# ucl-bug/helmnet

Hardware: AMD Instinct MI355X
Metric: solver iterations/sec (whole node), 256^2 domain batch=32 (higher is better)
Workload: dtype f32; 1 GPU; 256x256 ring-phantom SoS maps, batch=32 per GPU, point source [30, 128], shipped jcp checkpoint weights, UNet precision fp32 (BASELINE configs[1]); batch_per_gpu=32, domain=256, lanes=1, unet_precision=fp32, parallelism=dp1 (batch shards, no data-path collective)

## Files before the change

helmnet_amd/_lib.py:

```python
from __future__ import annotations

import ctypes
import os
from ctypes import POINTER, c_char_p, c_double, c_float, c_int, c_int64, c_size_t, c_void_p

import torch

_LIB_PATH = os.environ.get("HELMNET_HIP_LIB") or os.path.join(os.path.dirname(os.path.abspath(__file__)), "libhelmnet_hip.so")
_lib = None

HN_ACT = {"prelu": 0, "relu": 1, "leakyrelu": 2, "celu": 3, "tanh": 4, "gelu": 5, "tanhshrink": 6, "softplus": 7}
HN_PRECISION = {"fp32": 0, "bf16x3": 1, "fp16": 2, "bf16x2": 3, "valu": 4}
HN_OPTION = {"lanes": 0, "side_stream": 1, "deep": 3, "spectral_pfa": 4, "spectral_radix16": 5, "dc_valu": 6, "spectral_cols": 7, "train_fused": 10, "train_overlap": 11, "dc_pair": 12, "side_sync": 13, "state_kernel": 14, "hist_copy": 15, "inc_sigma_map": 16, "spectral_mixed": 17, "f64_fft": 18,
             "graph": 100, "train_lanes": 101, "spectral_plain": 102}
HN_COUNTER = {"graph_replays": 0, "eager_iterations": 1, "graphs_captured": 2, "stream_probes": 3, "side_candidate": 4, "train_fwd_events": 5, "flag_sync_iterations": 6, "spectral_route": 7, "f64_route": 8}
ABI_VERSION = 7
HN_VJP = {"continue": 1, "defer": 2}

SYMBOLS = {
    "hn_abi_version": (c_int, []),
    "hn_create": (c_int, [POINTER(c_void_p), c_int]),
    "hn_destroy": (None, [c_void_p]),
    "hn_last_error": (c_char_p, [c_void_p]),
    "hn_set_unet_precision": (c_int, [c_void_p, c_int]),
    "hn_get_unet_precision": (c_int, [c_void_p]),
    "hn_set_option": (c_int, [c_void_p, c_int, c_int]),
    "hn_get_counter": (c_int64, [c_void_p, c_int]),
    "hn_check_async_errors": (c_int, [c_void_p]),
    "hn_weight_count": (c_size_t, [c_int, c_int, c_int]),
    "hn_load_weights": (c_int, [c_void_p, POINTER(c_float), c_size_t, c_int, c_int, c_int, c_int]),
    "hn_set_domain": (c_int, [c_void_p, c_int, c_int, c_float, c_float]),
    "hn_set_domain_rect": (c_int, [c_void_p, c_int, c_int, c_int, c_float, c_float]),
    "hn_get_sigmas": (c_int, [c_void_p, c_void_p, c_void_p]),
    "hn_state_len": (c_int64, [c_void_p]),
    "hn_reserve": (c_int, [c_void_p, c_int]),
    "hn_laplacian": (c_int, [c_void_p, c_void_p, c_void_p, c_int, c_void_p]),
    "hn_residual": (c_int, [c_void_p, c_void_p, c_void_p, c_void_p, c_int, c_void_p, c_int, c_void_p]),
    "hn_residual_vjp": (c_int, [c_void_p, c_void_p, c_void_p, c_void_p, c_int, c_void_p]),
# ... 90 lines not shown
```

helmnet_amd/csrc/hn_api.hip:

```cpp
#include <cmath>
#include <cstdlib>
#include <cstring>

#include <cstdio>
#include "hn_internal.h"

namespace hn {

static thread_local std::string g_err;

void set_global_error(const char* msg) { g_err = msg; }

int fail(hn_ctx* ctx, int code, const char* fmt, ...) {
    char buf[512];
    va_list ap;
    va_start(ap, fmt);
    vsnprintf(buf, sizeof(buf), fmt, ap);
    va_end(ap);
    if (ctx) ctx->err = buf;
    g_err = buf;
    return code;
}

ProfScope::ProfScope(hn_ctx* ctx, int id, hipStream_t st) : c(ctx), s(st) {
// ... 270 lines not shown
    if (std::strncmp(prop.gcnArchName, "gfx950", 6) != 0)
        return fail(nullptr, HN_ERR_UNSUPPORTED, "device %d is %s; this library is built for gfx950 only", device_id, prop.gcnArchName);
    int prev = -1;
    (void)hipGetDevice(&prev);
    if ((e = hipSetDevice(device_id)) != hipSuccess) return fail(nullptr, HN_ERR_HIP, "hipSetDevice: %s", hipGetErrorString(e));
    if (prev >= 0 && prev != device_id) (void)hipSetDevice(prev);
    hn_ctx* c = new (std::nothrow) hn_ctx();
    if (!c) return fail(nullptr, HN_ERR_NOMEM, "out of host memory");
    c->device = device_id;
    *out = c;
    auto bad_env = [&](const char* name, const char* v) {
        const std::string why = c->err;
        hn_destroy(c);
        *out = nullptr;
        return fail(nullptr, HN_ERR_ARG, "hn_create: environment variable %s=%s rejected (%s)", name, v, why.c_str());
    };
    if (const char* v = getenv("HN_UNET_IMPL")) {
        const int mode = std::strcmp(v, "fp32") == 0 ? HN_PREC_FP32 : std::strcmp(v, "bf16x3") == 0 ? HN_PREC_BF16X3 : std::strcmp(v, "fp16") == 0 ? HN_PREC_FP16
                       : std::strcmp(v, "bf16x2") == 0 ? HN_PREC_BF16X2 : std::strcmp(v, "valu") == 0 ? HN_PREC_FP32_VALU : -1;
        if (hn_set_unet_precision(c, mode) != HN_OK) return bad_env("HN_UNET_IMPL", v);
    }
    const struct { const char* env; int opt; } knobs[] = {{"HN_STREAMS", HN_OPT_LANES}, {"HN_SIDE_STREAM", HN_OPT_SIDE_STREAM},
                                                            {"HN_GRAPH", HN_EXP_GRAPH}, {"HN_DEEP", HN_OPT_DEEP},
                                                            {"HN_TRAIN_LANES", HN_EXP_TRAIN_LANES}, {"HN_TRAIN_FUSED", HN_OPT_TRAIN_FUSED}, {"HN_TRAIN_OVERLAP", HN_OPT_TRAIN_OVERLAP}, {"HN_DC_VALU", HN_OPT_DC_VALU}, {"HN_DC_PAIR", HN_OPT_DC_PAIR}, {"HN_SIDE_SYNC", HN_OPT_SIDE_SYNC}, {"HN_STATE_KERNEL", HN_OPT_STATE_KERNEL}, {"HN_HIST_COPY", HN_OPT_HIST_COPY}, {"HN_INC_SIGMA_MAP", HN_OPT_INC_SIGMA_MAP}, {"HN_SPECTRAL_MIXED", HN_OPT_SPECTRAL_MIXED}, {"HN_F64_FFT", HN_OPT_F64_FFT}, {"HN_SPECTRAL_PLAIN", HN_EXP_SPECTRAL_PLAIN}};
    for (const char* name : {"ROCPROF_COUNTER_COLLECTION", "ROCPROF_COUNTERS", "ROCP_METRICS"})
        if (const char* v = getenv(name))
            if (v[0] != '\0' && std::strcmp(v, "0") != 0 && std::strcmp(v, "False") != 0 && std::strcmp(v, "false") != 0) c->opt_side_sync = 0;
    if (const char* v = getenv("HN_SIDE_PRIORITY")) { const int p = std::atoi(v); c->opt_side_priority = p < 0 || p > 3 ? 0 : p; }
    if (const char* v = getenv("HN_DEFER_JOIN")) c->opt_defer_join = std::atoi(v) != 0;
    for (const auto& k : knobs)
        if (const char* v = getenv(k.env)) {
            char* end = nullptr;
            const long n = std::strtol(v, &end, 10);
            if (end == v || *end != '\0') { c->err = "not an integer"; return bad_env(k.env, v); }
            if (hn_set_option(c, k.opt, (int)n) != HN_OK) return bad_env(k.env, v);
        }
    *out = c;
    return HN_OK;
}

int hn_set_unet_precision(hn_ctx* ctx, int precision) {
    if (!ctx) return HN_ERR_ARG;
    if (precision < HN_PREC_FP32 || precision > HN_PREC_FP32_VALU)
        return fail(ctx, HN_ERR_ARG, "hn_set_unet_precision: unknown mode %d", precision);
    if (precision != ctx->precision) clear_step_graphs(ctx);
    ctx->precision = precision;
    return HN_OK;
// ... 13 lines not shown
            ctx->opt_side_stream = value;
            break;
        case HN_EXP_GRAPH:
            if (value < 0 || value > 64 || (value > 1 && (value & 1)))
                return fail(ctx, HN_ERR_ARG, "HN_EXP_GRAPH must be 0, 1 or an even number of iterations per graph <= 64 (got %d)", value);
            ctx->opt_graph = value;
            break;
        case HN_OPT_DEEP:
            if (value < 0 || value > 2) return fail(ctx, HN_ERR_ARG, "HN_OPT_DEEP must be 0, 1 or 2 (got %d)", value);
            ctx->opt_deep = value;
            break;
        case HN_OPT_SPECTRAL_PFA:
            if (value < 0 || value > 1) return fail(ctx, HN_ERR_ARG, "HN_OPT_SPECTRAL_PFA must be 0 or 1 (got %d)", value);
            ctx->opt_pfa = value;
            break;
        case HN_OPT_SPECTRAL_MIXED:
            if (value < 0 || value > 1) return fail(ctx, HN_ERR_ARG, "HN_OPT_SPECTRAL_MIXED must be 0 or 1 (got %d)", value);
            ctx->opt_mixed = value;
            break;
        case HN_OPT_F64_FFT:
            if (value < 0 || value > 1) return fail(ctx, HN_ERR_ARG, "HN_OPT_F64_FFT must be 0 or 1 (got %d)", value);
            ctx->opt_f64_fft = value;
            break;
        case HN_OPT_DC_VALU:
            if (value < 0 || value > 4) return fail(ctx, HN_ERR_ARG, "HN_OPT_DC_VALU must be 0 .. 4 (got %d)", value);
            ctx->opt_dc_valu = value;
            break;
        case HN_OPT_DC_PAIR:
            if (value < 0 || value > 1) return fail(ctx, HN_ERR_ARG, "HN_OPT_DC_PAIR must be 0 or 1 (got %d)", value);
            ctx->opt_dc_pair = value;
            break;
        case HN_OPT_STATE_KERNEL:
            if (value < 0 || value > 1) return fail(ctx, HN_ERR_ARG, "HN_OPT_STATE_KERNEL must be 0 or 1 (got %d)", value);
            ctx->opt_state_kernel = value;
            break;
        case HN_OPT_INC_SIGMA_MAP:
            if (value < 0 || value > 1) return fail(ctx, HN_ERR_ARG, "HN_OPT_INC_SIGMA_MAP must be 0 or 1 (got %d)", value);
            ctx->opt_inc_sigma_map = value;
            break;
        case HN_OPT_HIST_COPY:
            if (value < 0 || value > 1) return fail(ctx, HN_ERR_ARG, "HN_OPT_HIST_COPY must be 0 or 1 (got %d)", value);
            ctx->opt_hist_copy = value;
            break;
        case HN_OPT_SIDE_SYNC:
            if (value < 0 || value > 1) return fail(ctx, HN_ERR_ARG, "HN_OPT_SIDE_SYNC must be 0 or 1 (got %d)", value);
            ctx->opt_side_sync = value;
// ... 20 lines not shown
            break;
        case HN_OPT_TRAIN_OVERLAP:
            if (value < 0 || value > 2) return fail(ctx, HN_ERR_ARG, "HN_OPT_TRAIN_OVERLAP must be 0, 1 or 2 (got %d)", value);
            ctx->opt_train_overlap = value;
            break;
        default: return fail(ctx, HN_ERR_ARG, "hn_set_option: unknown option %d", option);
    }
    clear_step_graphs(ctx);
    return HN_OK;
}

int64_t hn_get_counter(const hn_ctx* ctx, int counter) {
    if (!ctx) return -1;
    switch (counter) {
        case HN_CNT_GRAPH_REPLAYS: return ctx->graph_replays;
        case HN_CNT_EAGER_ITERATIONS: return ctx->eager_iterations;
        case HN_CNT_GRAPHS_CAPTURED: return ctx->graphs_captured;
        case HN_CNT_STREAM_PROBES: return ctx->probes_run;
        case HN_CNT_TRAIN_FWD_EVENTS: return ctx->train_fwd_events;
        case HN_CNT_FLAG_SYNC_ITERATIONS: return ctx->flag_sync_iterations;
        case HN_CNT_SIDE_CANDIDATE: return ctx->picks[0].known.empty() ? -1 : ctx->picks[0].last_chosen;
        case HN_CNT_SPECTRAL_ROUTE: return ctx->rect != nullptr ? 5 : ctx->tab.n == 0 ? 0 : ctx->tab.pow2 ? 1 : ctx->tab.pfa_p != 0 ? 2 : ctx->tab.mix_p != 0 ? 4 : 3;
        case HN_CNT_F64_ROUTE: return ctx->f64_route;
        default: return -1;
    }
}

void hn_destroy(hn_ctx* ctx) {
    if (!ctx) return;
    DeviceGuard guard(ctx);
    (void)hipDeviceSynchronize();
    clear_step_graphs(ctx);
    if (ctx->cap_stream) (void)hipStreamDestroy(ctx->cap_stream);
    (void)hipFree(ctx->it_counter);
    free_workspace(ctx);
    train_free(ctx);
    unet_f64_free(ctx);
    jvp_free(ctx);
    krylov_free(ctx);
    f64_fft_free(ctx);
    spec_free(ctx->tab);
    spec_rect_free(ctx);
    spec_lossy_free(ctx);
    (void)hipFree(ctx->wdev);
    (void)hipFree(ctx->fragdev);
    for (int j = 0; j < ctx->n_streams; ++j) {
// ... 297 lines not shown

int hn_double_conv(hn_ctx* ctx, const float* x, int cin, int cout, const float* weights_host, int act_kind, float* out,
                   int batch, int h, int w, void* stream) {
    if (!ctx || !x || !weights_host || !out) return fail(ctx, HN_ERR_ARG, "hn_double_conv: NULL argument");
    if (batch < 1 || h < 1 || w < 1) return fail(ctx, HN_ERR_ARG, "hn_double_conv: batch, h, w must be positive");
    if (act_kind < HN_ACT_PRELU || act_kind > HN_ACT_SOFTPLUS) return fail(ctx, HN_ERR_UNSUPPORTED, "activation kind %d is not implemented", act_kind);
    const bool ok = (cout == kFeat && (cin == kInCh || cin == kFeat || cin == kFeat + kState || cin == 2 * kFeat)) || (cout == kState && cin == kFeat + kState);
    if (!ok) return fail(ctx, HN_ERR_UNSUPPORTED, "hn_double_conv: (cin, cout) = (%d, %d) is not one of (6,8) (8,8) (10,8) (16,8) (10,2)", cin, cout);
    DcW dw;
    size_t n_floats = 0;
    const RawDc r = raw_dc(n_floats, cin, cout, cout);
    return with_temp_weights(ctx, n_floats, (hipStream_t)stream,
        [&](std::vector<float>& packed, float* dev) { dw = pack_dc(weights_host, packed.data(), dev, r, act_kind); },
        [&]() { return module_double_conv(ctx, x, cin, cout, dw, out, batch, h, w, (hipStream_t)stream); });
}

int hn_conv8x8(hn_ctx* ctx, const float* x, const float* weights_host, int transposed, float* out, int batch, int h, int w, void* stream) {
    if (!ctx || !x || !weights_host || !out) return fail(ctx, HN_ERR_ARG, "hn_conv8x8: NULL argument");
    if (batch < 1 || h < 1 || w < 1) return fail(ctx, HN_ERR_ARG, "hn_conv8x8: batch, h, w must be positive");
    if (!transposed && ((h | w) & 1)) return fail(ctx, HN_ERR_UNSUPPORTED, "hn_conv8x8: the stride-2 convolution needs even h, w (got %d, %d)", h, w);
    K8W kw;
    size_t n_floats = 0;
    const RawK8 r = raw_k8(n_floats);
    return with_temp_weights(ctx, n_floats, (hipStream_t)stream,
        [&](std::vector<float>& packed, float* dev) { kw = pack_k8(weights_host, packed.data(), dev, r, transposed != 0); },
        [&]() { return module_conv8x8(ctx, x, kw, transposed != 0, out, batch, h, w, (hipStream_t)stream); });
}

int hn_out_conv(hn_ctx* ctx, const float* x, const float* weights_host, float* out, int batch, int h, int w, void* stream) {
    if (!ctx || !x || !weights_host || !out) return fail(ctx, HN_ERR_ARG, "hn_out_conv: NULL argument");
    if (batch < 1 || h < 1 || w < 1) return fail(ctx, HN_ERR_ARG, "hn_out_conv: batch, h, w must be positive");
    const float *dw = nullptr, *db = nullptr;
    return with_temp_weights(ctx, 2 * kFeat + 2, (hipStream_t)stream,
        [&](std::vector<float>& packed, float* dev) {
            repack_oihw(weights_host, packed.data(), 2, kFeat, 1);
            packed[2 * kFeat] = weights_host[2 * kFeat]; packed[2 * kFeat + 1] = weights_host[2 * kFeat + 1];
            dw = dev; db = dev + 2 * kFeat;
        },
        [&]() { return module_out_conv(ctx, x, dw, db, out, batch, h, w, (hipStream_t)stream); });
}

}

namespace hn {
namespace {

struct StepArgs {
    float *wf, *res, *states;
    const float *k_sq, *src;
// ... 397 lines not shown
```

helmnet_amd/csrc/hn_internal.h:

```cpp
#pragma once
#include <hip/hip_runtime.h>

#include <complex>
#include <cstdarg>
#include <cstdint>
#include <cstdio>
#include <string>
#include <vector>

#include "helmnet_hip.h"

namespace hn {

constexpr int kFeat = 8;
constexpr int kCounterStride = 32;
constexpr int kState = 2;
constexpr int kInCh = 6;
constexpr int kMaxDepth = 6;

struct Src {
    const float* p;
    long sb;
    long sc;
    float scale;
// ... 219 lines not shown
    long pair_flags_cap = 0;
    unsigned pair_epoch = 0;
    unsigned* pair_done = nullptr;
    int opt_hist_copy = 0;
    int opt_state_kernel = 1;
    int opt_side_sync = 1;
    unsigned* sync_flags = nullptr;
    unsigned sync_epoch = 0;
    int* sync_err = nullptr;
    int* sync_err_dev = nullptr;
    hn_stream_verdict_rec* stream_tab = nullptr;
    hn_stream_verdict_rec* stream_tab_dev = nullptr;
    int stream_tab_cap = 0;
    float2* inc_sigma_map = nullptr;
    int inc_sigma_band = 0;
    float inc_w_sigma[144]{};
    int opt_inc_sigma_map = 1;
    const float* zero_page = nullptr;
    const float* outc_w = nullptr;
    const float* outc_b = nullptr;
    hn::SpecTables tab;
    hn::F64Fft* f64fft = nullptr;
    int opt_f64_fft = 0;
    int f64_route = 0;
    hn::RectDomain* rect = nullptr;
    hn::RectAxis* lossy_axis = nullptr;
    struct Geometry {
        int h = 0, w = 0;
        const float* sigmas = nullptr;
        long plane() const { return (long)h * w; }
    } geo;
    int64_t state_len = 0;
    int64_t state_off[hn::kMaxDepth]{};
    int cap_batch = 0;
    float* buf_a[hn::kMaxDepth + 1]{};
    float* buf_o[hn::kMaxDepth]{};
    float* buf_y[hn::kMaxDepth + 1]{};
    float* st_tmp = nullptr;
    struct SideLane {
        hipStream_t stream = nullptr; hipEvent_t ev[hn::kMaxDepth]{}; hipEvent_t done = nullptr;
        bool pending = false;
    };
    SideLane side[8];
    struct SidePick {
        hipStream_t cand[4]{};
        struct Known { hipStream_t ref[3]{}; int nref = 0; int chosen = 0; };
// ... 200 lines not shown
    const float* a2;
    const float* z; long z_sb, z_sc;
    float* gz; long gz_sb, gz_sc;
    const float* slope; int act;
    double* slope_part;
    McBwdDst dst[3];
};
struct McBwdAux {
    const float* g; long g_sb, g_sc;
    const float* a1;
    const float* a2;
    const float* z; long z_sb, z_sc;
    float* gz; long gz_sb, gz_sc;
    const float* slope; double* slope_part;
    McBwdDst dst;
};
int launch_dc8_bwd_aux(hn_ctx* ctx, const McBwd& a, const McBwdAux& x, int H, int W, int batch, hipStream_t s);
bool dc8_bwd_applies(int H, int W);
int dc8_bwd_tiles(int H, int W, int batch);
int launch_dc8_bwd(hn_ctx* ctx, const McBwd& a, int cin, int H, int W, int batch, hipStream_t s);
void launch_dc8_tape(DcKind kind, Src a, Src b, Src c, Dst out, const float* frag1, const float* b1, const float* slope, const float* frag2,
                    const float* b2, int act, float* z, int H, int W, int batch, hipStream_t s);
void launch_down(const hn_ctx* ctx, Src in, Dst out, const K8Frag& w, int Hin, int Win, int batch, hipStream_t s,
                 SyncHook hook = SyncHook{});
void launch_up(const hn_ctx* ctx, Src in, Dst out, const K8Frag& w, int Hin, int Win, int batch, hipStream_t s, bool accumulate = false,
               SyncHook hook = SyncHook{});

void pack_valu_q(const float* w_oihw, int cin, float* dst);
void pack_outc3x3_valu(const float* w2, const float* wo, float* dst);
bool dc_valu_applies(const hn_ctx* ctx, int act, Src a, Src b, Src c, DcKind kind, int H, int W);
void launch_dc_valu(const hn_ctx* ctx, DcKind kind, Src a, Src b, Src c, Dst out, const DcW& w, const FinalEpi* fin, int H, int W, int batch, hipStream_t s);

void pack_dca(const float* w_oihw, int cin, const float* scale, float* dst);
bool dc_asm_applies(const hn_ctx* ctx, int act, Src a, Src b, Src c, DcKind kind, int H, int W);
void launch_dc_asm(const hn_ctx* ctx, DcKind kind, Src a, Src b, Src c, Dst out, const DcW& w, const FinalEpi* fin, int H, int W, int batch, hipStream_t s);
struct StateLevel { Src a, b; Dst out; DcW w; int H, W; };
bool conv_state_applies(const hn_ctx* ctx, const StateLevel& v);
void launch_conv_state(const hn_ctx* ctx, int n, const StateLevel* lv, int batch, hipStream_t s);
bool dc_asm_pair_applies(const hn_ctx* ctx, Src wf, Src res, Src sig, Src x0, Src st, int H, int W, int batch, int ws_off);
void launch_dc_asm_pair(hn_ctx* ctx, Src wf, Src res, Src sig, Dst x0_out, Src x0, Src st, Dst out0, int H, int W, int batch, int ws_off, bool capturing, hipStream_t s);

void pack_frag_3x3_c2(const float* w_oihw, int cin, float* dst);
bool deep_applies(const hn_ctx* ctx);
int launch_deep(hn_ctx* ctx, const float* x_in, long x_sb, const float* st_in, float* st_out, long st_sb, long st_sc, float* y_out,
                long y_sb, int batch, hipStream_t s, SyncHook hook = SyncHook{});

void pack_frag_down2(const float* w_oihw, float* dst);
// ... 3 lines not shown
struct UnetCall {
    Src wf{}, res{}, sig{};
    const float* states_in = nullptr; float* states_out = nullptr;
    float* d_out = nullptr;
    float* wf_out = nullptr; const float* wf_in = nullptr;
    int batch = 0, ws_off = 0;
    hipStream_t stream = nullptr;
    hipEvent_t after_down0 = nullptr;
    hn_ctx::SideLane* side_lane = nullptr;
    bool defer_join = false;
};
int unet_forward(hn_ctx* ctx, const UnetCall& c);
int side_join(hn_ctx* ctx, hn_ctx::SideLane* side_lane, hipStream_t s);
bool side_flags_apply(hn_ctx* ctx, hipStream_t s);
int ensure_sync_words(hn_ctx* ctx);
int build_inc_sigma_map(hn_ctx* ctx);
int check_async(hn_ctx* ctx, const char* who);
int zero_async(hn_ctx* ctx, void* p, size_t bytes, hipStream_t s);
void launch_sync_gate(hn_ctx* ctx, const unsigned* flag, unsigned epoch, hipStream_t s);
void launch_sync_signal(unsigned* flag, unsigned epoch, hipStream_t s);
int side_stream_for(hn_ctx* ctx, int slot, const hipStream_t* refs, int nrefs, bool may_sync, hipStream_t* out);

int module_double_conv(hn_ctx* ctx, const float* x, int cin, int cout, const DcW& w, float* out, int batch, int H, int W, hipStream_t s);
int module_conv8x8(hn_ctx* ctx, const float* x, const K8W& w, bool transposed, float* out, int batch, int H, int W, hipStream_t s);
int module_out_conv(hn_ctx* ctx, const float* x, const float* w_io, const float* b, float* out, int batch, int H, int W, hipStream_t s);

}
```

helmnet_amd/csrc/hn_mfma.hip:

```cpp
#include <cstdlib>

#include "hn_internal.h"
#include <cstring>
#include <cstdint>

namespace hn {
namespace {

typedef float f32x4 __attribute__((ext_vector_type(4)));
typedef float f32x2 __attribute__((ext_vector_type(2)));

constexpr int cdiv_(int a, int b) { return (a + b - 1) / b; }
constexpr int cmax_(int a, int b) { return a > b ? a : b; }

__device__ __forceinline__ f32x4 mfma4(float a, float b, f32x4 c) {
    return __builtin_amdgcn_mfma_f32_16x16x4f32(a, b, c, 0, 0, 0);
}
__device__ __forceinline__ float div1000(float x) {
    const float r = 1e-3f;
    const float qv = x * r;
    const float e = fmaf(-qv, 1000.0f, x);
    return fmaf(e, r, qv);
}
template <int N>
// ... 1776 lines not shown
                for (int wr = 0; wr < C::NWIN; ++wr) bv[(kx + 1) & 1][wr] = t[bbase + 2 * wr * C::PI + kx + 1];
            }
#pragma unroll
            for (int wr = 0; wr < C::NWIN; ++wr) acc[wr] = mfma4(afrag[kx], bv[kx & 1][wr], acc[wr]);
            interleave_mfma_dsread<C::NWIN>();
            __builtin_amdgcn_sched_barrier(0);
        }
    }
    const int X = X0 + 16 * wx + n;
    const float b0 = bias[2 * q], b1 = bias[2 * q + 1];
    if (X < Wout) {
#pragma unroll
        for (int r = 0; r < C::R; ++r) {
            const int Y = Y0 + wy * C::R + r;
            if (Y < Hout) {
                float* p = out.p + (long)b * out.sb + (long)(2 * q) * out.sc + (long)Y * Wout + X;
                p[0] = acc[r][0] + acc[r + 2][1] + b0;
                p[out.sc] = acc[r][2] + acc[r + 2][3] + b1;
            }
        }
    }
}

template <int WX, int R_>
struct UpCfg2 {
    static constexpr int WY = 4 / WX;
    static constexpr int R = R_;
    static constexpr int TH = R * WY, TW = 16 * WX;
    static constexpr int IR = TH + 3;
    static constexpr int IC = TW + 4;
    static constexpr int PI = ((IC + 15) / 32) * 32 + 16;
    static constexpr int PLANE = IR * PI;
    static constexpr int PLANE_P = PLANE + 64;
    static constexpr int NT = 256;
    static constexpr int NL = cdiv_(IR * IC, NT);
};

template <int WX, int R_, bool ALL, bool ACC = false>
__global__ __launch_bounds__(256, 3) void k_up_mfma(Src in, Dst out, const float* __restrict__ afr ,
                                                  const float* __restrict__ bias, int Hin, int Win, SyncHook hook) {
    using C = UpCfg2<WX, R_>;
    __shared__ float lds[(ALL ? kFeat : 4) * C::PLANE_P];
    sync_hook_begin(hook);
    const int tid = threadIdx.x, lane = tid & 63;
    const int wave = __builtin_amdgcn_readfirstlane(tid >> 6);
    const int n = lane & 15, q = lane >> 4;
// ... 570 lines not shown
    else launch_dc8_bwd_n<2>(a, H, W, batch, s);
    HN_HIP(ctx, hipGetLastError());
    return HN_OK;
}

int launch_dc8_bwd_aux(hn_ctx* ctx, const McBwd& a, const McBwdAux& x, int H, int W, int batch, hipStream_t s) {
    if (!dc8_bwd_applies(H, W) || a.dst[0].nch != kFeat || a.dst[1].nch != kFeat || x.dst.nch != kState)
        return fail(ctx, HN_ERR_ARG, "internal: the decoder + hidden-state backward kernel needs channel groups 8 | 8 and 2");
    int tw, tx, ty;
    dc8_bwd_shape(H, W, tw, tx, ty);
    const int nt = tx * ty * batch;
    const bool gen = a.act > HN_ACT_LEAKYRELU;
    if (tw == 32) {
        if (gen) hipLaunchKernelGGL((k_dc_bwd_mfma_aux<8, 32, true>), dim3(nt), dim3(256), 0, s, a, x, H, W, tx, ty, nt);
        else hipLaunchKernelGGL((k_dc_bwd_mfma_aux<8, 32, false>), dim3(nt), dim3(256), 0, s, a, x, H, W, tx, ty, nt);
    } else {
        if (gen) hipLaunchKernelGGL((k_dc_bwd_mfma_aux<8, 16, true>), dim3(nt), dim3(256), 0, s, a, x, H, W, tx, ty, nt);
        else hipLaunchKernelGGL((k_dc_bwd_mfma_aux<8, 16, false>), dim3(nt), dim3(256), 0, s, a, x, H, W, tx, ty, nt);
    }
    HN_HIP(ctx, hipGetLastError());
    return HN_OK;
}

void launch_down(const hn_ctx* ctx, Src in, Dst out, const K8Frag& w, int Hin, int Win, int batch, hipStream_t s, SyncHook hook) {
    const int Wout = Win / 2, Hout = Hin / 2;
    const float *frag = w.f32, *bias = w.bias;
    const int mode = w.f16 != nullptr ? ctx->precision : HN_PREC_FP32;
    if ((mode == HN_PREC_FP16 || mode == HN_PREC_BF16X2) && Wout >= 64) {
        const dim3 g(cdiv_(Wout, 16), cdiv_(Hout, 16), batch);
        if (mode == 3) hipLaunchKernelGGL((k_down_x16<SplitBf16x2>), g, dim3(256), 0, s, in, out, w.bf16, bias, Hin, Win);
        else hipLaunchKernelGGL((k_down_x16<HalfF16>), g, dim3(256), 0, s, in, out, w.f16, bias, Hin, Win);
        return;
    }
    if (Wout > 64) hipLaunchKernelGGL((k_down_mfma<4, false>), dim3(cdiv_(Wout, 64), cdiv_(Hout, 16), batch), dim3(256), 0, s, in, out, frag, bias, Hin, Win, hook);
    else if (Wout > 32) {
        const dim3 g(cdiv_(Wout, 32), cdiv_(Hout, 16), batch);
        hipLaunchKernelGGL((k_down_mfma<2, false>), g, dim3(256), 0, s, in, out, frag, bias, Hin, Win, hook);
    }
    else {
        const dim3 g(cdiv_(Wout, 16), cdiv_(Hout, 16), batch);
        hipLaunchKernelGGL((k_down_mfma<1, true>), g, dim3(256), 0, s, in, out, frag, bias, Hin, Win, hook);
    }
}

void launch_up(const hn_ctx* ctx, Src in, Dst out, const K8Frag& w, int Hin, int Win, int batch, hipStream_t s, bool accumulate, SyncHook hook) {
    const float *frag = w.f32, *bias = w.bias;
    const int mode = w.f16 != nullptr ? ctx->precision : HN_PREC_FP32;
    if (mode >= HN_PREC_BF16X3 && mode <= HN_PREC_BF16X2 && Win >= 64) {
        const dim3 g(cdiv_(Win, 16), cdiv_(Hin + 1, 20), batch);
// ... 19 lines not shown
```

helmnet_amd/csrc/hn_unet.hip:

```cpp
#include "hn_internal.h"

namespace hn {
namespace {

constexpr int cdiv(int a, int b) { return (a + b - 1) / b; }

template <int CA, int CB, int CC, int CM, int CO, int TW>
struct DcCfg {
    static constexpr int TH = 16;
    static constexpr int CIN = CA + CB + CC;
    static constexpr int IR = TH + 4;
    static constexpr int PI = TW + 4;
    static constexpr int MR = TH + 2;
    static constexpr int S1 = cdiv(TW + 2, 4);
    static constexpr int PM = S1 * 4;
    static constexpr int S2 = TW / 4;
    static constexpr int NT = cdiv(S1 * MR, 64) * 64;
    static constexpr int PLANE = IR * PI;
    static constexpr int NL = cdiv(PLANE, NT);
    static_assert(CA % 2 == 0 && CB % 2 == 0 && CC % 2 == 0, "sources are staged two channels at a time");
};

struct DcEpi {
    const float* ow;
// ... 373 lines not shown
    auto plane = [&](int d) { return (long)(H >> d) * (W >> d); };
    auto feat = [&](float* p, int d) { return Dst{p + (long)ws_off * kFeat * plane(d), kFeat * plane(d), plane(d)}; };
    auto featsrc = [&](const float* p, int d) { return Src{p + (long)ws_off * kFeat * plane(d), kFeat * plane(d), plane(d), 1.f}; };
    auto st_old = [&](int d) { return Src{c.states_in + ctx->state_off[d], 2 * L, L, 1.f}; };
    auto state_level = [&](int d) {
        return StateLevel{featsrc(ctx->buf_o[d], d), st_old(d), Dst{c.states_out + ctx->state_off[d], 2 * L, L}, ctx->st[d].w, H >> d, W >> d};
    };
    auto dc = [&](DcKind kind, int d, Src a, Src b, Src c3, Dst out, const FinalEpi* fin) {
        const DcLayer& l = kind == DcKind::Inc ? ctx->inc : kind == DcKind::Signal ? ctx->sig[d] : ctx->dec[d];
        const int h = H >> d, w = W >> d;
        if (mfma) return launch_dc8(ctx, kind, a, b, c3, out, l, fin, h, w, batch, s);
        switch (kind) {
            case DcKind::Inc: launch_dc<2, 2, 2, kFeat, kFeat, 0>(a, b, c3, out, l.w, noepi, h, w, batch, s); break;
            case DcKind::Signal: launch_dc<kFeat, kState, 0, kFeat, kFeat, 0>(a, b, c3, out, l.w, noepi, h, w, batch, s); break;
            case DcKind::Bottleneck: launch_dc<kFeat, 0, 0, kFeat, kFeat, 0>(a, b, c3, out, l.w, noepi, h, w, batch, s); break;
            case DcKind::Decoder:
                if (fin == nullptr) launch_dc<kFeat, kFeat, 0, kFeat, kFeat, 0>(a, b, c3, out, l.w, noepi, h, w, batch, s);
                else launch_dc<kFeat, kFeat, 0, kFeat, kFeat, 1>(a, b, c3, out, l.w, DcEpi{ctx->outc_w, ctx->outc_b, fin->d_out, fin->wf_out, fin->wf_in}, h, w, batch, s);
                break;
        }
    };
    auto down = [&](int d) {
        const int h = H >> d, w = W >> d;
        if (mfma) launch_down(ctx, featsrc(ctx->buf_o[d], d), feat(ctx->buf_a[d + 1], d + 1), ctx->down[d].f, h, w, batch, s);
        else hipLaunchKernelGGL(k_down8x8, dim3(cdiv(w / 2, DownCfg::TW), cdiv(h / 2, DownCfg::TH), batch), dim3(DownCfg::NT), 0, s,
                                featsrc(ctx->buf_o[d], d), feat(ctx->buf_a[d + 1], d + 1), ctx->down[d].w, h, w);
    };
    auto up = [&](int d, const SyncHook& hook) {
        const int h = H >> (d + 1), w = W >> (d + 1);
        if (mfma) launch_up(ctx, featsrc(ctx->buf_y[d + 1], d + 1), feat(ctx->buf_a[d], d), ctx->up[d].f, h, w, batch, s, false, hook);
        else hipLaunchKernelGGL(k_up8x8, dim3(cdiv(w, UpCfg::TW), cdiv(h, UpCfg::TH), batch), dim3(UpCfg::NT), 0, s,
                                featsrc(ctx->buf_y[d + 1], d + 1), feat(ctx->buf_a[d], d), ctx->up[d].w, h, w);
    };
    auto conv_state = [&](const StateLevel& v, hipStream_t st) {
        if (conv_state_applies(ctx, v)) launch_conv_state(ctx, 1, &v, batch, st);
        else launch_dc<kFeat, kState, 0, kState, kState, 0>(v.a, v.b, none, v.out, v.w, noepi, v.H, v.W, batch, st);
    };

    hipStreamCaptureStatus cs = hipStreamCaptureStatusNone;
    const bool not_capturing = hipStreamIsCapturing(s, &cs) == hipSuccess && cs == hipStreamCaptureStatusNone;
    (void)hipGetLastError();
    const bool eager = not_capturing && ws_off == 0 && ctx->opt_lanes == 1 && side_lane != nullptr;
    const bool pair = mfma && dc_asm_pair_applies(ctx, c.wf, c.res, c.sig, featsrc(ctx->buf_a[0], 0), st_old(0), H, W, batch, ws_off);
    if (pair) {
        if (side_lane != nullptr) {
            int rc = side_join(ctx, side_lane, s);
            if (rc != HN_OK) return rc;
// ... 152 lines not shown
        a1 = fmaf(w[c * 2 + 1], v, a1);
    }
    out[b * 2 * plane + p] = a0;
    out[(b * 2 + 1) * plane + p] = a1;
}
}

int module_double_conv(hn_ctx* ctx, const float* x, int cin, int cout, const DcW& w, float* out, int batch, int H, int W, hipStream_t s) {
    const long plane = (long)H * W;
    const DcEpi noepi{nullptr, nullptr, nullptr, nullptr};
    const Src none{nullptr, 0, 0, 1.f};
    auto view = [&](int c0) { return Src{x + c0 * plane, cin * plane, plane, 1.f}; };
    const Dst o{out, cout * plane, plane};
    if (cin == 6 && cout == kFeat) launch_dc<2, 2, 2, kFeat, kFeat, 0>(view(0), view(2), view(4), o, w, noepi, H, W, batch, s);
    else if (cin == kFeat && cout == kFeat) launch_dc<kFeat, 0, 0, kFeat, kFeat, 0>(view(0), none, none, o, w, noepi, H, W, batch, s);
    else if (cin == kFeat + kState && cout == kFeat) launch_dc<kFeat, kState, 0, kFeat, kFeat, 0>(view(0), view(kFeat), none, o, w, noepi, H, W, batch, s);
    else if (cin == 2 * kFeat && cout == kFeat) launch_dc<kFeat, kFeat, 0, kFeat, kFeat, 0>(view(0), view(kFeat), none, o, w, noepi, H, W, batch, s);
    else if (cin == kFeat + kState && cout == kState) launch_dc<kFeat, kState, 0, kState, kState, 0>(view(0), view(kFeat), none, o, w, noepi, H, W, batch, s);
    else return fail(ctx, HN_ERR_UNSUPPORTED, "hn_double_conv: (cin, cout) = (%d, %d) is not one of (6,8) (8,8) (10,8) (16,8) (10,2)", cin, cout);
    HN_HIP(ctx, hipGetLastError());
    return HN_OK;
}

int module_conv8x8(hn_ctx* ctx, const float* x, const K8W& w, bool transposed, float* out, int batch, int H, int W, hipStream_t s) {
    const long pin = (long)H * W;
    const Src in{x, kFeat * pin, pin, 1.f};
    if (!transposed) {
        const long po = (long)(H / 2) * (W / 2);
        hipLaunchKernelGGL(k_down8x8, dim3(cdiv(W / 2, DownCfg::TW), cdiv(H / 2, DownCfg::TH), batch), dim3(DownCfg::NT), 0, s, in,
                           Dst{out, kFeat * po, po}, w, H, W);
    } else {
        const long po = 4 * pin;
        hipLaunchKernelGGL(k_up8x8, dim3(cdiv(W, UpCfg::TW), cdiv(H, UpCfg::TH), batch), dim3(UpCfg::NT), 0, s, in, Dst{out, kFeat * po, po}, w, H, W);
    }
    HN_HIP(ctx, hipGetLastError());
    return HN_OK;
}

int module_out_conv(hn_ctx* ctx, const float* x, const float* w_io, const float* b, float* out, int batch, int H, int W, hipStream_t s) {
    const long plane = (long)H * W, total = plane * batch;
    hipLaunchKernelGGL(k_out_conv, dim3((unsigned)((total + 255) / 256)), dim3(256), 0, s, x, w_io, b, out, plane, total);
    HN_HIP(ctx, hipGetLastError());
    return HN_OK;
}

}
```

include/helmnet_hip.h:

```cpp
#ifndef HELMNET_HIP_H
#define HELMNET_HIP_H

#include <stddef.h>
#include <stdint.h>

#ifdef __cplusplus
extern "C" {
#endif

typedef struct hn_ctx hn_ctx;

enum hn_status {
    HN_OK = 0,
    HN_ERR_ARG = -1,
    HN_ERR_STATE = -2,
    HN_ERR_UNSUPPORTED = -3,
    HN_ERR_HIP = -4,
    HN_ERR_NOMEM = -5
};

enum hn_act { HN_ACT_PRELU = 0, HN_ACT_RELU = 1, HN_ACT_LEAKYRELU = 2, HN_ACT_CELU = 3, HN_ACT_TANH = 4, HN_ACT_GELU = 5,
              HN_ACT_TANHSHRINK = 6, HN_ACT_SOFTPLUS = 7 };

enum hn_precision { HN_PREC_FP32 = 0, HN_PREC_BF16X3 = 1, HN_PREC_FP16 = 2, HN_PREC_BF16X2 = 3, HN_PREC_FP32_VALU = 4 };

enum hn_option {
    HN_OPT_LANES = 0,
    HN_OPT_SIDE_STREAM = 1,
    HN_OPT_DEEP = 3,
    HN_OPT_SPECTRAL_PFA = 4,
    HN_OPT_SPECTRAL_MIXED = 17,
    HN_OPT_F64_FFT = 18,
    HN_OPT_SPECTRAL_RADIX16 = 5,
    HN_OPT_DC_VALU = 6,
    HN_OPT_DC_PAIR = 12,
    HN_OPT_SIDE_SYNC = 13,
    HN_OPT_STATE_KERNEL = 14,
    HN_OPT_HIST_COPY = 15,
    HN_OPT_INC_SIGMA_MAP = 16,
    HN_OPT_SPECTRAL_COLS = 7,
    HN_OPT_TRAIN_FUSED = 10,
    HN_OPT_TRAIN_OVERLAP = 11,
    HN_EXP_GRAPH = 100,
    HN_EXP_TRAIN_LANES = 101,
    HN_EXP_SPECTRAL_PLAIN = 102
};
enum hn_counter { HN_CNT_GRAPH_REPLAYS = 0,
                  HN_CNT_EAGER_ITERATIONS = 1,
                  HN_CNT_GRAPHS_CAPTURED = 2,
                  HN_CNT_STREAM_PROBES = 3,
                  HN_CNT_SIDE_CANDIDATE = 4,
                  HN_CNT_TRAIN_FWD_EVENTS = 5,
                  HN_CNT_FLAG_SYNC_ITERATIONS = 6,
                  HN_CNT_SPECTRAL_ROUTE = 7,
                  HN_CNT_F64_ROUTE = 8 };

#define HN_ABI_VERSION 7
int hn_abi_version(void);

int hn_create(hn_ctx** out, int device_id);
void hn_destroy(hn_ctx* ctx);
const char* hn_last_error(const hn_ctx* ctx);

size_t hn_weight_count(int features, int depth, int state_ch);

int hn_load_weights(hn_ctx* ctx, const float* blob, size_t n_floats, int features, int depth,
                    int state_ch, int act_kind);

int hn_set_unet_precision(hn_ctx* ctx, int precision);
int hn_get_unet_precision(const hn_ctx* ctx);
int hn_set_option(hn_ctx* ctx, int option, int value);
int64_t hn_get_counter(const hn_ctx* ctx, int counter);
int hn_check_async_errors(hn_ctx* ctx);

int hn_set_domain(hn_ctx* ctx, int n, int pml, float sigma_max, float k);

int hn_set_domain_rect(hn_ctx* ctx, int h, int w, int pml, float sigma_max, float k);

// ... 115 lines not shown
```

Before: 2251 iterations/s.

## Add K-split MFMA kernel for fp32 downsampling conv at 64-wide output

```diff
diff --git a/helmnet_amd/_lib.py b/helmnet_amd/_lib.py
--- a/helmnet_amd/_lib.py
+++ b/helmnet_amd/_lib.py
@@ -11,9 +11,9 @@
 
 HN_ACT = {"prelu": 0, "relu": 1, "leakyrelu": 2, "celu": 3, "tanh": 4, "gelu": 5, "tanhshrink": 6, "softplus": 7}
 HN_PRECISION = {"fp32": 0, "bf16x3": 1, "fp16": 2, "bf16x2": 3, "valu": 4}
-HN_OPTION = {"lanes": 0, "side_stream": 1, "deep": 3, "spectral_pfa": 4, "spectral_radix16": 5, "dc_valu": 6, "spectral_cols": 7, "train_fused": 10, "train_overlap": 11, "dc_pair": 12, "side_sync": 13, "state_kernel": 14, "hist_copy": 15, "inc_sigma_map": 16, "spectral_mixed": 17, "f64_fft": 18,
+HN_OPTION = {"lanes": 0, "side_stream": 1, "deep": 3, "spectral_pfa": 4, "spectral_radix16": 5, "dc_valu": 6, "spectral_cols": 7, "train_fused": 10, "train_overlap": 11, "dc_pair": 12, "side_sync": 13, "state_kernel": 14, "hist_copy": 15, "inc_sigma_map": 16, "spectral_mixed": 17, "f64_fft": 18, "mid_ksplit": 19,
              "graph": 100, "train_lanes": 101, "spectral_plain": 102}
-HN_COUNTER = {"graph_replays": 0, "eager_iterations": 1, "graphs_captured": 2, "stream_probes": 3, "side_candidate": 4, "train_fwd_events": 5, "flag_sync_iterations": 6, "spectral_route": 7, "f64_route": 8}
+HN_COUNTER = {"graph_replays": 0, "eager_iterations": 1, "graphs_captured": 2, "stream_probes": 3, "side_candidate": 4, "train_fwd_events": 5, "flag_sync_iterations": 6, "spectral_route": 7, "f64_route": 8, "mid_ksplit": 9}
 ABI_VERSION = 7
 HN_VJP = {"continue": 1, "defer": 2}
 
diff --git a/helmnet_amd/csrc/hn_api.hip b/helmnet_amd/csrc/hn_api.hip
--- a/helmnet_amd/csrc/hn_api.hip
+++ b/helmnet_amd/csrc/hn_api.hip
@@ -316,7 +316,7 @@
     }
     const struct { const char* env; int opt; } knobs[] = {{"HN_STREAMS", HN_OPT_LANES}, {"HN_SIDE_STREAM", HN_OPT_SIDE_STREAM},
                                                             {"HN_GRAPH", HN_EXP_GRAPH}, {"HN_DEEP", HN_OPT_DEEP},
-                                                            {"HN_TRAIN_LANES", HN_EXP_TRAIN_LANES}, {"HN_TRAIN_FUSED", HN_OPT_TRAIN_FUSED}, {"HN_TRAIN_OVERLAP", HN_OPT_TRAIN_OVERLAP}, {"HN_DC_VALU", HN_OPT_DC_VALU}, {"HN_DC_PAIR", HN_OPT_DC_PAIR}, {"HN_SIDE_SYNC", HN_OPT_SIDE_SYNC}, {"HN_STATE_KERNEL", HN_OPT_STATE_KERNEL}, {"HN_HIST_COPY", HN_OPT_HIST_COPY}, {"HN_INC_SIGMA_MAP", HN_OPT_INC_SIGMA_MAP}, {"HN_SPECTRAL_MIXED", HN_OPT_SPECTRAL_MIXED}, {"HN_F64_FFT", HN_OPT_F64_FFT}, {"HN_SPECTRAL_PLAIN", HN_EXP_SPECTRAL_PLAIN}};
+                                                            {"HN_TRAIN_LANES", HN_EXP_TRAIN_LANES}, {"HN_TRAIN_FUSED", HN_OPT_TRAIN_FUSED}, {"HN_TRAIN_OVERLAP", HN_OPT_TRAIN_OVERLAP}, {"HN_DC_VALU", HN_OPT_DC_VALU}, {"HN_DC_PAIR", HN_OPT_DC_PAIR}, {"HN_SIDE_SYNC", HN_OPT_SIDE_SYNC}, {"HN_STATE_KERNEL", HN_OPT_STATE_KERNEL}, {"HN_HIST_COPY", HN_OPT_HIST_COPY}, {"HN_INC_SIGMA_MAP", HN_OPT_INC_SIGMA_MAP}, {"HN_SPECTRAL_MIXED", HN_OPT_SPECTRAL_MIXED}, {"HN_F64_FFT", HN_OPT_F64_FFT}, {"HN_MID_KSPLIT", HN_OPT_MID_KSPLIT}, {"HN_SPECTRAL_PLAIN", HN_EXP_SPECTRAL_PLAIN}};
     for (const char* name : {"ROCPROF_COUNTER_COLLECTION", "ROCPROF_COUNTERS", "ROCP_METRICS"})
         if (const char* v = getenv(name))
             if (v[0] != '\0' && std::strcmp(v, "0") != 0 && std::strcmp(v, "False") != 0 && std::strcmp(v, "false") != 0) c->opt_side_sync = 0;
@@ -376,6 +376,10 @@
             if (value < 0 || value > 1) return fail(ctx, HN_ERR_ARG, "HN_OPT_F64_FFT must be 0 or 1 (got %d)", value);
             ctx->opt_f64_fft = value;
             break;
+        case HN_OPT_MID_KSPLIT:
+            if (value < 0 || value > 1) return fail(ctx, HN_ERR_ARG, "HN_OPT_MID_KSPLIT must be 0 or 1 (got %d)", value);
+            ctx->opt_mid_ksplit = value;
+            break;
         case HN_OPT_DC_VALU:
             if (value < 0 || value > 4) return fail(ctx, HN_ERR_ARG, "HN_OPT_DC_VALU must be 0 .. 4 (got %d)", value);
             ctx->opt_dc_valu = value;
@@ -442,6 +446,7 @@
         case HN_CNT_SIDE_CANDIDATE: return ctx->picks[0].known.empty() ? -1 : ctx->picks[0].last_chosen;
         case HN_CNT_SPECTRAL_ROUTE: return ctx->rect != nullptr ? 5 : ctx->tab.n == 0 ? 0 : ctx->tab.pow2 ? 1 : ctx->tab.pfa_p != 0 ? 2 : ctx->tab.mix_p != 0 ? 4 : 3;
         case HN_CNT_F64_ROUTE: return ctx->f64_route;
+        case HN_CNT_MID_KSPLIT: return ctx->mid_ksplit_launches;
         default: return -1;
     }
 }
@@ -785,9 +790,17 @@
     K8W kw;
     size_t n_floats = 0;
     const RawK8 r = raw_k8(n_floats);
+    const long pin = (long)h * w;
+    const bool ksplit = !transposed && down_ksplit_applies(ctx, Src{x, kFeat * pin, pin, 1.f}, h, w);
+    const size_t frag_off = n_floats;
+    if (ksplit) n_floats += (size_t)kFeat * kFeat * 64;
+    const float* frag = nullptr;
     return with_temp_weights(ctx, n_floats, (hipStream_t)stream,
-        [&](std::vector<float>& packed, float* dev) { kw = pack_k8(weights_host, packed.data(), dev, r, transposed != 0); },
-        [&]() { return module_conv8x8(ctx, x, kw, transposed != 0, out, batch, h, w, (hipStream_t)stream); });
+        [&](std::vector<float>& packed, float* dev) {
+            kw = pack_k8(weights_host, packed.data(), dev, r, transposed != 0);
+            if (ksplit) { pack_frag_down(weights_host + r.w, packed.data() + frag_off); frag = dev + frag_off; }
+        },
+        [&]() { return module_conv8x8(ctx, x, kw, transposed != 0, out, batch, h, w, (hipStream_t)stream, frag); });
 }
 
 int hn_out_conv(hn_ctx* ctx, const float* x, const float* weights_host, float* out, int batch, int h, int w, void* stream) {
diff --git a/helmnet_amd/csrc/hn_internal.h b/helmnet_amd/csrc/hn_internal.h
--- a/helmnet_amd/csrc/hn_internal.h
+++ b/helmnet_amd/csrc/hn_internal.h
@@ -265,6 +265,8 @@
     hn::SpecTables tab;
     hn::F64Fft* f64fft = nullptr;
     int opt_f64_fft = 0;
+    int opt_mid_ksplit = 1;
+    mutable long mid_ksplit_launches = 0;
     int f64_route = 0;
     hn::RectDomain* rect = nullptr;
     hn::RectAxis* lossy_axis = nullptr;
@@ -511,7 +513,8 @@
 void launch_dc8_tape(DcKind kind, Src a, Src b, Src c, Dst out, const float* frag1, const float* b1, const float* slope, const float* frag2,
                     const float* b2, int act, float* z, int H, int W, int batch, hipStream_t s);
 void launch_down(const hn_ctx* ctx, Src in, Dst out, const K8Frag& w, int Hin, int Win, int batch, hipStream_t s,
-                 SyncHook hook = SyncHook{});
+                 SyncHook hook = SyncHook{}, bool ksplit = false);
+bool down_ksplit_applies(const hn_ctx* ctx, Src in, int Hin, int Win);
 void launch_up(const hn_ctx* ctx, Src in, Dst out, const K8Frag& w, int Hin, int Win, int batch, hipStream_t s, bool accumulate = false,
                SyncHook hook = SyncHook{});
 
@@ -561,7 +564,7 @@
 int side_stream_for(hn_ctx* ctx, int slot, const hipStream_t* refs, int nrefs, bool may_sync, hipStream_t* out);
 
 int module_double_conv(hn_ctx* ctx, const float* x, int cin, int cout, const DcW& w, float* out, int batch, int H, int W, hipStream_t s);
-int module_conv8x8(hn_ctx* ctx, const float* x, const K8W& w, bool transposed, float* out, int batch, int H, int W, hipStream_t s);
+int module_conv8x8(hn_ctx* ctx, const float* x, const K8W& w, bool transposed, float* out, int batch, int H, int W, hipStream_t s, const float* frag_ks = nullptr);
 int module_out_conv(hn_ctx* ctx, const float* x, const float* w_io, const float* b, float* out, int batch, int H, int W, hipStream_t s);
 
 }
diff --git a/helmnet_amd/csrc/hn_mfma.hip b/helmnet_amd/csrc/hn_mfma.hip
--- a/helmnet_amd/csrc/hn_mfma.hip
+++ b/helmnet_amd/csrc/hn_mfma.hip
@@ -1822,6 +1822,121 @@
     }
 }
 
+struct DnKs {
+    static constexpr int TH = 8, TW = 16;
+    static constexpr int NWIN = TH + 2;
+    static constexpr int IR = 2 * TH + 6;
+    static constexpr int IC4 = (2 * TW + 8) / 4;
+    static constexpr int PI = 4 * IC4 + 1;
+    static constexpr int PLANE = IR * PI;
+    static constexpr int NT = 256;
+    static constexpr int NV = IR * IC4;
+    static_assert(NV <= NT, "one staging thread per float4 of a plane");
+    static constexpr int RED = 4 * TH * 2 * 64;
+    static constexpr int LDS_FLOATS = cmax_(kFeat * PLANE, RED);
+};
+
+__global__ __launch_bounds__(256, 4) void k_down_ks(Src in, Dst out, const float* __restrict__ afr ,
+                                                    const float* __restrict__ bias, int Hin, int Win) {
+    using C = DnKs;
+    __shared__ float lds[C::LDS_FLOATS];
+    const int tid = threadIdx.x, lane = tid & 63;
+    const int wave = __builtin_amdgcn_readfirstlane(tid >> 6);
+    const int n = lane & 15, q = lane >> 4;
+    const TileId tl = xcd_tile();
+    const int b = tl.z;
+    const int X0 = tl.x * C::TW, Y0 = tl.y * C::TH;
+    const int Hout = Hin / 2, Wout = Win / 2;
+    const float* const base = in.p + (long)b * in.sb;
+
+    float afrag[2][8];
+#pragma unroll
+    for (int c = 0; c < 2; ++c)
+#pragma unroll
+        for (int kx = 0; kx < 8; ++kx) afrag[c][kx] = afr[((2 * wave + c) * 8 + kx) * 64 + lane];
+    {
+        const int ir = tid / C::IC4, ic4 = tid - ir * C::IC4;
+        const int y = 2 * Y0 - 3 + ir, x = 2 * X0 - 4 + 4 * ic4;
+        const bool inr = tid < C::NV;
+        const bool ok = inr && y >= 0 && y < Hin && x >= 0 && x < Win;
+        float4 st[kFeat];
+#pragma unroll
+        for (int c = 0; c < kFeat; ++c) st[c] = make_float4(0.f, 0.f, 0.f, 0.f);
+        if (ok) {
+            const float* const src = base + (long)y * Win + x;
+#pragma unroll
+            for (int c = 0; c < kFeat; ++c) st[c] = *reinterpret_cast<const float4*>(src + (long)c * in.sc);
+        }
+        if (inr) {
+            float* const t = lds + ir * C::PI + 4 * ic4;
+#pragma unroll
+            for (int c = 0; c < kFeat; ++c) {
+                t[c * C::PLANE] = st[c].x; t[c * C::PLANE + 1] = st[c].y; t[c * C::PLANE + 2] = st[c].z; t[c * C::PLANE + 3] = st[c].w;
+            }
+        }
+    }
+    __syncthreads();
+
+    const float* const t0 = lds + 2 * wave * C::PLANE + q * C::PI + 2 * n + 1;
+    f32x4 acc[C::NWIN];
+#pragma unroll
+    for (int i = 0; i < C::NWIN; ++i) acc[i] = (f32x4){0.f, 0.f, 0.f, 0.f};
+    float bv[2][C::NWIN][2];
+#pragma unroll
+    for (int wr = 0; wr < C::NWIN; ++wr) {
+        bv[0][wr][0] = t0[2 * wr * C::PI];
+        bv[0][wr][1] = t0[2 * wr * C::PI + 1];
+    }
+    __builtin_amdgcn_sched_barrier(0);
+#pragma unroll
+    for (int st = 0; st < 8; ++st) {
+        const int c = st / 4, kx = 2 * (st % 4);
+        if (st + 1 < 8) {
+            const int o1 = ((st + 1) / 4) * C::PLANE + 2 * ((st + 1) % 4);
+#pragma unroll
+            for (int wr = 0; wr < C::NWIN; ++wr) {
+                bv[(st + 1) & 1][wr][0] = t0[o1 + 2 * wr * C::PI];
+                bv[(st + 1) & 1][wr][1] = t0[o1 + 2 * wr * C::PI + 1];
+            }
+        }
+#pragma unroll
+        for (int j = 0; j < 2; ++j)
+#pragma unroll
+            for (int wr = 0; wr < C::NWIN; ++wr) acc[wr] = mfma4(afrag[c][kx + j], bv[st & 1][wr][j], acc[wr]);
+#pragma unroll
+        for (int i = 0; i < C::NWIN; ++i) {
+            __builtin_amdgcn_sched_group_barrier(0x008, 2, 0);
+            __builtin_amdgcn_sched_group_barrier(0x100, 1, 0);
+        }
+        __builtin_amdgcn_sched_barrier(0);
+    }
+
+    __syncthreads();
+#pragma unroll
+    for (int r = 0; r < C::TH; ++r) {
+        lds[((wave * C::TH + r) * 2 + 0) * 64 + lane] = acc[r][0] + acc[r + 2][1];
+        lds[((wave * C::TH + r) * 2 + 1) * 64 + lane] = acc[r][2] + acc[r + 2][3];
+    }
+    __syncthreads();
+    const int X = X0 + n;
+    const float b0 = bias[2 * q], b1 = bias[2 * q + 1];
+#pragma unroll
+    for (int rr = 0; rr < 2; ++rr) {
+        const int r = 2 * wave + rr, Y = Y0 + r;
+        float s[2];
+#pragma unroll
+        for (int j = 0; j < 2; ++j) {
+            const float* p = lds + (r * 2 + j) * 64 + lane;
+            s[j] = (p[0] + p[C::TH * 128]) + (p[2 * C::TH * 128] + p[3 * C::TH * 128]);
+        }
+        if (Y < Hout) {
+            float* p = out.p + (long)b * out.sb + (long)(2 * q) * out.sc + (long)Y * Wout + X;
+            p[0] = s[0] + b0;
+            p[out.sc] = s[1] + b1;
+        }
+    }
+}
+
 template <int WX, int R_>
 struct UpCfg2 {
     static constexpr int WY = 4 / WX;
@@ -2438,9 +2553,20 @@
     return HN_OK;
 }
 
-void launch_down(const hn_ctx* ctx, Src in, Dst out, const K8Frag& w, int Hin, int Win, int batch, hipStream_t s, SyncHook hook) {
+bool down_ksplit_applies(const hn_ctx* ctx, Src in, int Hin, int Win) {
+    const int Wout = Win / 2;
+    const bool aligned = (reinterpret_cast<uintptr_t>(in.p) & 15) == 0 && ((in.sb | in.sc) & 3) == 0;
+    return (ctx->opt_mid_ksplit & 1) && ctx->precision == HN_PREC_FP32 && Wout == 64 && !(Hin & 1) && aligned;
+}
+
+void launch_down(const hn_ctx* ctx, Src in, Dst out, const K8Frag& w, int Hin, int Win, int batch, hipStream_t s, SyncHook hook, bool ksplit) {
     const int Wout = Win / 2, Hout = Hin / 2;
     const float *frag = w.f32, *bias = w.bias;
+    if (ksplit && hook.store == nullptr && hook.wait == nullptr && down_ksplit_applies(ctx, in, Hin, Win)) {
+        hipLaunchKernelGGL(k_down_ks, dim3(cdiv_(Wout, DnKs::TW), cdiv_(Hout, DnKs::TH), batch), dim3(256), 0, s, in, out, frag, bias, Hin, Win);
+        ++ctx->mid_ksplit_launches;
+        return;
+    }
     const int mode = w.f16 != nullptr ? ctx->precision : HN_PREC_FP32;
     if ((mode == HN_PREC_FP16 || mode == HN_PREC_BF16X2) && Wout >= 64) {
         const dim3 g(cdiv_(Wout, 16), cdiv_(Hout, 16), batch);
diff --git a/helmnet_amd/csrc/hn_unet.hip b/helmnet_amd/csrc/hn_unet.hip
--- a/helmnet_amd/csrc/hn_unet.hip
+++ b/helmnet_amd/csrc/hn_unet.hip
@@ -419,7 +419,7 @@
     };
     auto down = [&](int d) {
         const int h = H >> d, w = W >> d;
-        if (mfma) launch_down(ctx, featsrc(ctx->buf_o[d], d), feat(ctx->buf_a[d + 1], d + 1), ctx->down[d].f, h, w, batch, s);
+        if (mfma) launch_down(ctx, featsrc(ctx->buf_o[d], d), feat(ctx->buf_a[d + 1], d + 1), ctx->down[d].f, h, w, batch, s, SyncHook{}, true);
         else hipLaunchKernelGGL(k_down8x8, dim3(cdiv(w / 2, DownCfg::TW), cdiv(h / 2, DownCfg::TH), batch), dim3(DownCfg::NT), 0, s,
                                 featsrc(ctx->buf_o[d], d), feat(ctx->buf_a[d + 1], d + 1), ctx->down[d].w, h, w);
     };
@@ -618,12 +618,13 @@
     return HN_OK;
 }
 
-int module_conv8x8(hn_ctx* ctx, const float* x, const K8W& w, bool transposed, float* out, int batch, int H, int W, hipStream_t s) {
+int module_conv8x8(hn_ctx* ctx, const float* x, const K8W& w, bool transposed, float* out, int batch, int H, int W, hipStream_t s, const float* frag_ks) {
     const long pin = (long)H * W;
     const Src in{x, kFeat * pin, pin, 1.f};
     if (!transposed) {
         const long po = (long)(H / 2) * (W / 2);
-        hipLaunchKernelGGL(k_down8x8, dim3(cdiv(W / 2, DownCfg::TW), cdiv(H / 2, DownCfg::TH), batch), dim3(DownCfg::NT), 0, s, in,
+        if (frag_ks != nullptr) launch_down(ctx, in, Dst{out, kFeat * po, po}, K8Frag{frag_ks, nullptr, nullptr, w.b}, H, W, batch, s, SyncHook{}, true);
+        else hipLaunchKernelGGL(k_down8x8, dim3(cdiv(W / 2, DownCfg::TW), cdiv(H / 2, DownCfg::TH), batch), dim3(DownCfg::NT), 0, s, in,
                            Dst{out, kFeat * po, po}, w, H, W);
     } else {
         const long po = 4 * pin;
diff --git a/include/helmnet_hip.h b/include/helmnet_hip.h
--- a/include/helmnet_hip.h
+++ b/include/helmnet_hip.h
@@ -31,6 +31,7 @@
     HN_OPT_SPECTRAL_PFA = 4,
     HN_OPT_SPECTRAL_MIXED = 17,
     HN_OPT_F64_FFT = 18,
+    HN_OPT_MID_KSPLIT = 19,
     HN_OPT_SPECTRAL_RADIX16 = 5,
     HN_OPT_DC_VALU = 6,
     HN_OPT_DC_PAIR = 12,
@@ -53,7 +54,8 @@
                   HN_CNT_TRAIN_FWD_EVENTS = 5,
                   HN_CNT_FLAG_SYNC_ITERATIONS = 6,
                   HN_CNT_SPECTRAL_ROUTE = 7,
-                  HN_CNT_F64_ROUTE = 8 };
+                  HN_CNT_F64_ROUTE = 8,
+                  HN_CNT_MID_KSPLIT = 9 };
 
 #define HN_ABI_VERSION 7
 int hn_abi_version(void);
```

After: 2259 iterations/s (median of 6 runs). No clear change (+0.4%).
